# waczjoan/gaussian-mesh-splatting

Hardware: AMD Instinct MI355X
Metric: train iters/s (fwd+bwd raster) @800×800, 300k Gaussians; HBM GB/s vs roofline (higher is better)
Workload: dtype f32

## Files before the change

### gaussian-mesh-splatting_amd/csrc/binning.hip

```cpp
#include "gms_blend.h"
#include "gms_common.h"
#include "gms_forward.h"

namespace gms {

constexpr int SORT_RUN = 1024;
constexpr int SORT_RUNS_PER_TILE = 8;
constexpr int SORT_BIG_CHUNK = SORT_RUN * SORT_RUNS_PER_TILE;
constexpr int MP_CHUNK = 1024;

constexpr int NSCAN = 11;
constexpr int NCLASS = 6;
constexpr int SCAN_THREADS = 1024;

__device__ __forceinline__ void tile_terms(uint32_t c, uint32_t L, uint32_t t[NSCAN], int sort_np = 0)
{
    const uint32_t ns = max(1u, (c + L - 1) / L);
    t[0] = c; t[1] = ns; t[2] = ns > 1 ? ns : 0;
    const uint32_t r = c % L;
    t[3] = c / L;
    t[4] = r * 4 >= 3 * L ? 1u : 0u;
    t[5] = (r * 4 < 3 * L && r * 2 >= L) ? 1u : 0u;
    t[6] = (r * 2 < L && r * 4 >= L) ? 1u : 0u;
    t[7] = (r * 4 < L && r != 0) ? 1u : 0u;
// ... 177 lines not shown
    if (lane == WAVE - 1) s_wave[wave] = incl;
    __syncthreads();
    uint32_t pre = incl - sum;
    for (int w = 0; w < wave; w++) pre += s_wave[w];
#pragma unroll
    for (int k = 0; k < 16; k++)
        if (k < per && b + k < e) { s_off[b + k] = pre; pre += c[k]; }
    if (tid == BLOCK - 1) s_off[T] = pre;
    __syncthreads();
}

struct InlineScanLds {
    uint32_t chunk[NSCAN][BLOCK];
    uint32_t wave_tot[NSCAN][BLOCK / WAVE];
    uint32_t total[NSCAN];
    uint32_t wave_deep[BLOCK / WAVE];
    uint32_t deepest;
};

__device__ __forceinline__ void inline_scan_build(const uint32_t *count, int T, uint32_t L, int sort_np, InlineScanLds &S)
{
    const int tid = threadIdx.x, lane = tid & 63, wave = tid >> 6;
    const int per = (T + BLOCK - 1) / BLOCK;
    const int b = min(T, tid * per), e = min(T, b + per);
    uint32_t run[NSCAN];
    uint32_t deepest = 0;
#pragma unroll
    for (int k = 0; k < NSCAN; k++) run[k] = 0;
    for (int t = b; t < e; t++) {
        uint32_t q[NSCAN];
        tile_terms(count[t], L, q, sort_np);
        deepest = max(deepest, q[0]);
#pragma unroll
        for (int k = 0; k < NSCAN; k++) run[k] += q[k];
    }
    for (int d = 32; d >= 1; d >>= 1) deepest = max(deepest, (uint32_t)__shfl_xor((int)deepest, d));
    if (lane == 0) S.wave_deep[wave] = deepest;
    uint32_t incl[NSCAN];
#pragma unroll
    for (int k = 0; k < NSCAN; k++) {
        incl[k] = wave_incl_scan_u32(run[k], lane);
        if (lane == WAVE - 1) S.wave_tot[k][wave] = incl[k];
    }
    __syncthreads();
#pragma unroll
    for (int k = 0; k < NSCAN; k++) {
        uint32_t pre = incl[k] - run[k];
        for (int w = 0; w < wave; w++) pre += S.wave_tot[k][w];
        S.chunk[k][tid] = pre;
    }
    if (tid == 0) {
#pragma unroll
        for (int k = 0; k < NSCAN; k++) S.total[k] = S.wave_tot[k][0] + S.wave_tot[k][1] + S.wave_tot[k][2] + S.wave_tot[k][3];
        S.deepest = max(max(S.wave_deep[0], S.wave_deep[1]), max(S.wave_deep[2], S.wave_deep[3]));
    }
    __syncthreads();
}

struct InlineScanArgs {
    const uint32_t *count;
    uint32_t *offset, *unit_first, *mseg_first, *class_first, *scan_out;
    uint32_t L;
};

template <bool INLINE>
__global__ void __launch_bounds__(BLOCK) emit_instances_kernel(int P, int gx, int gy, const int *radii, GeomState geom,
                                                               const uint32_t *tile_offset, uint32_t *tile_cursor,
                                                               uint64_t *keys, uint64_t capacity, unsigned emit_blocks, FillUnitsArgs fu,
                                                               int32_t *host_slot, int32_t seq, const uint32_t *scan_out, InlineScanArgs is)
{
    constexpr int OFFW = INLINE ? INLINE_SCAN_MAX_T + 4 : 0;
    __shared__ uint32_t smem[OFFW + 3 * TT_SLOTS + BLOCK / WAVE];
    static_assert(sizeof(InlineScanLds) <= sizeof(uint32_t) * (INLINE_SCAN_MAX_T + 4 + 3 * TT_SLOTS), "spare blocks alias the emit blocks' LDS");
    uint32_t *s_off = smem, *s_wave = smem + OFFW + 3 * TT_SLOTS;
    const unsigned nspare = gridDim.x - emit_blocks;
    const bool spare = INLINE ? blockIdx.x < nspare : blockIdx.x >= emit_blocks;
    const unsigned spare_idx = INLINE ? blockIdx.x : blockIdx.x - emit_blocks;
    const unsigned emit_idx = INLINE ? blockIdx.x - nspare : blockIdx.x;
    if (spare) {
        if (INLINE) {
            InlineScanLds &S = *reinterpret_cast<InlineScanLds *>(smem);
            const int T = fu.T;
            inline_scan_build(is.count, T, is.L, fu.sort_np, S);
            const int t = (int)spare_idx * BLOCK + (int)threadIdx.x;
            if (spare_idx == 0 && threadIdx.x == 0) {
                is.scan_out[0] = S.total[0]; is.scan_out[1] = S.deepest; is.scan_out[2] = S.total[1]; is.scan_out[3] = is.L;
                if (host_slot) publish_counts(host_slot, seq, S.total[0], S.deepest, S.total[1]);
                is.offset[T] = S.total[0]; is.unit_first[T] = S.total[1]; is.mseg_first[T] = S.total[2];
#pragma unroll
                for (int k = 0; k < NCLASS + 2; k++) is.class_first[k * (T + 1) + T] = S.total[3 + k];
            }
            if (t < T) {
                const int per = (T + BLOCK - 1) / BLOCK;
                const int c0 = t / per;
                uint32_t pre[NSCAN], tot[NSCAN];
#pragma unroll
                for (int k = 0; k < NSCAN; k++) { pre[k] = S.chunk[k][c0]; tot[k] = S.total[k]; }
                for (int u = c0 * per; u < t; u++) {
                    uint32_t q[NSCAN];
                    tile_terms(is.count[u], is.L, q, fu.sort_np);
#pragma unroll
                    for (int k = 0; k < NSCAN; k++) pre[k] += q[k];
                }
                is.offset[t] = pre[0]; is.unit_first[t] = pre[1]; is.mseg_first[t] = pre[2];
#pragma unroll
                for (int k = 0; k < NCLASS + 2; k++) is.class_first[k * (T + 1) + t] = pre[3 + k];
                fill_units_tile(fu, t, is.count[t], is.L, pre, tot);
            }
            return;
        }
        if (spare_idx == 0 && threadIdx.x == 0 && host_slot) publish_counts(host_slot, seq, scan_out[0], scan_out[1], scan_out[2]);
        fill_units(fu, (int)spare_idx);
        return;
    }
    if (INLINE) { inline_offsets(is.count, fu.T, s_off, s_wave); tile_offset = s_off; }
    const int i = (int)emit_idx * BLOCK + threadIdx.x;
    const ushort4 rc = i < P ? geom.rect[i] : make_ushort4(0, 0, 0, 0);
    const uint32_t dbits = i < P ? __float_as_uint(geom.depth[i]) : 0u;
    const int minx = rc.x, miny = rc.y, maxx = rc.z, maxy = rc.w;
    const int rw = maxx - minx;
    const int area = rw * (maxy - miny);
    const uint64_t key = area > 0 ? (((uint64_t)dbits << 32) | (uint32_t)i) : 0ull;
    (void)radii; (void)gy;
    const bool small = area <= SMALL_AREA;
    const int lane = threadIdx.x & 63;
    int cx = minx, cy = miny;
    int *tt_key = reinterpret_cast<int *>(smem + OFFW);
    uint32_t *tt_cnt = smem + OFFW + TT_SLOTS, *tt_base = smem + OFFW + 2 * TT_SLOTS;
    for (int q = threadIdx.x; q < TT_SLOTS; q += BLOCK) { tt_key[q] = -1; tt_cnt[q] = 0; }
    __syncthreads();
    if (small) {
        for (int k = 0; k < area; k++) {
            const int sl = tt_insert(tt_key, cy * gx + cx);
            if (sl >= 0) atomicAdd(&tt_cnt[sl], 1u);
            if (++cx == maxx) { cx = minx; cy++; }
        }
    }
    __syncthreads();
    for (int q = threadIdx.x; q < TT_SLOTS; q += BLOCK)
        if (tt_key[q] >= 0) {
            tt_base[q] = tile_offset[tt_key[q]] + atomicAdd(&tile_cursor[tt_key[q]], tt_cnt[q]);
            tt_cnt[q] = 0;
        }
    __syncthreads();
    if (small) {
        cx = minx; cy = miny;
        for (int k = 0; k < area; k++) {
            const int t = cy * gx + cx;
            const int sl = tt_find(tt_key, t);
            const uint64_t slot = sl >= 0 ? (uint64_t)tt_base[sl] + atomicAdd(&tt_cnt[sl], 1u)
                                          : (uint64_t)tile_offset[t] + atomicAdd(&tile_cursor[t], 1u);
            if (slot < capacity) keys[slot] = key;
            if (++cx == maxx) { cx = minx; cy++; }
        }
    }
    uint64_t big = __ballot(!small);
    while (big) {
        const int src = __builtin_ctzll(big);
        big &= big - 1;
        const int bminx = __builtin_amdgcn_readlane(minx, src), bminy = __builtin_amdgcn_readlane(miny, src);
        const int brw = __builtin_amdgcn_readlane(rw, src), barea = __builtin_amdgcn_readlane(area, src);
        const uint32_t klo = (uint32_t)__builtin_amdgcn_readlane((int)(uint32_t)key, src);
        const uint32_t khi = (uint32_t)__builtin_amdgcn_readlane((int)(uint32_t)(key >> 32), src);
        const uint64_t bkey = ((uint64_t)khi << 32) | klo;
        for (int k = lane; k < barea; k += WAVE) {
            const int ty = k / brw, tx = k - ty * brw;
            const int t = (bminy + ty) * gx + bminx + tx;
            const uint64_t slot = (uint64_t)tile_offset[t] + atomicAdd(&tile_cursor[t], 1u);
            if (slot < capacity) keys[slot] = bkey;
        }
    }
}

__device__ __forceinline__ void ce(uint64_t &x, uint64_t &y)
{
    if (x > y) { uint64_t t = x; x = y; y = t; }
}


constexpr int WAVE_SPAN = 128;

template <int THREADS>
__device__ __forceinline__ void stage_sync(int span, int &prev_span)
{
    if (span > WAVE_SPAN || prev_span > WAVE_SPAN) __syncthreads();
    else wave_sync();
    prev_span = span;
}

template <int THREADS>
__device__ void lds_bitonic(uint64_t *s, int m, int k0, int j0, bool first_mirror, int tid)
{
    int prev = 1 << 30;
    for (int k = k0, lk = 31 - __builtin_clz(k0); k <= m; k <<= 1, lk++) {
        const int hk = k >> 1;
        if (k > k0 || first_mirror) {
            stage_sync<THREADS>(k, prev);
            for (int i = tid; i < (m >> 1); i += THREADS) {
                const int blk = i >> (lk - 1), off = i & (hk - 1);
                const int lo = (blk << lk) + off, hi = (blk << lk) + k - 1 - off;
                ce(s[lo], s[hi]);
            }
        }
        int j = (k > k0 || first_mirror) ? (k >> 2) : j0;
        for (int lj = j > 0 ? 31 - __builtin_clz(j) : 0; j >= 1; j >>= 1, lj--) {
            stage_sync<THREADS>(2 * j, prev);
            for (int i = tid; i < (m >> 1); i += THREADS) {
                const int lo = ((i >> lj) << (lj + 1)) + (i & (j - 1));
                ce(s[lo], s[lo + j]);
            }
        }
    }
    __syncthreads();
}


enum { SORT_SINGLE = 0, SORT_LDS, SORT_MERGEPATH, SORT_FALLBACK };

__host__ __device__ __forceinline__ int sort_passes(uint64_t n)
{
    const uint64_t runs = (n + SORT_RUN - 1) / SORT_RUN;
    int q = 0;
    while ((1ull << q) < runs) q++;
    return q;
}

__device__ __forceinline__ int sort_class(uint64_t n, int passes_launched, int &q)
{
    q = 0;
    if (n <= (uint64_t)SORT_RUN) return SORT_SINGLE;
    q = sort_passes(n);
    if (q <= passes_launched) return SORT_MERGEPATH;
    return n <= (uint64_t)SORT_BIG_CHUNK ? SORT_LDS : SORT_FALLBACK;
}

template <int CTRL>
__device__ __forceinline__ uint64_t dpp64(uint64_t v)
{
    const int lo = __builtin_amdgcn_update_dpp(0, (int)(uint32_t)v, CTRL, 0xf, 0xf, false);
    const int hi = __builtin_amdgcn_update_dpp(0, (int)(uint32_t)(v >> 32), CTRL, 0xf, 0xf, false);
    return ((uint64_t)(uint32_t)hi << 32) | (uint32_t)lo;
}
template <int ML>
__device__ __forceinline__ uint64_t lane_xor64(uint64_t v)
{
    if (ML == 1) return dpp64<0xB1>(v);
    if (ML == 2) return dpp64<0x4E>(v);
    if (ML == 3) return dpp64<0x1B>(v);
    if (ML == 4) return dpp64<0x1B>(dpp64<0x141>(v));
    if (ML == 7) return dpp64<0x141>(v);
    if (ML == 8) return dpp64<0x128>(v);
    if (ML == 15) return dpp64<0x140>(v);
    const int lo = __shfl_xor((int)(uint32_t)v, ML), hi = __shfl_xor((int)(uint32_t)(v >> 32), ML);
    return ((uint64_t)(uint32_t)hi << 32) | (uint32_t)lo;
}

template <int M>
__device__ __forceinline__ void sort_step(uint64_t (&k)[4], int t, uint64_t *lds)
{
    constexpr int MR = M & 3, ML = (M >> 2) & 63, MW = M >> 8;
    constexpr int TOP = M >= 512 ? 512 : M >= 256 ? 256 : M >= 128 ? 128 : M >= 64 ? 64 : M >= 32 ? 32 : M >= 16 ? 16 : M >= 8 ? 8 : M >= 4 ? 4 : M >= 2 ? 2 : 1;
    if (ML == 0 && MW == 0) {
        if (MR == 1) { ce(k[0], k[1]); ce(k[2], k[3]); }
        else if (MR == 2) { ce(k[0], k[2]); ce(k[1], k[3]); }
        else { ce(k[0], k[3]); ce(k[1], k[2]); }
        return;
    }
    uint64_t p[4];
    if (MW != 0) {
        __syncthreads();
#pragma unroll
        for (int r = 0; r < 4; r++) lds[4 * t + r] = k[r];
        __syncthreads();
#pragma unroll
        for (int r = 0; r < 4; r++) p[r] = lds[(4 * t + r) ^ M];
    } else {
#pragma unroll
        for (int r = 0; r < 4; r++) p[r] = lane_xor64<ML>(k[r ^ MR]);
    }
    const bool keep_min = ((4 * t) & TOP) == 0;
#pragma unroll
    for (int r = 0; r < 4; r++) {
        const bool less = p[r] < k[r];
        k[r] = (less == keep_min) ? p[r] : k[r];
    }
}
template <int J>
__device__ __forceinline__ void sort_half_cleaners(uint64_t (&k)[4], int t, uint64_t *lds)
{
    if constexpr (J >= 1) {
        sort_step<J>(k, t, lds);
        sort_half_cleaners<J / 2>(k, t, lds);
    }
}
template <int K>
__device__ __forceinline__ void sort_level(uint64_t (&k)[4], int t, uint64_t *lds)
{
    sort_step<K - 1>(k, t, lds);
    sort_half_cleaners<K / 4>(k, t, lds);
}

__global__ void __launch_bounds__(256) tile_presort_reg_kernel(const uint32_t *tile_offset, const uint32_t *run_total, const uint2 *run_tab,
                                                           uint32_t max_runs, uint64_t *keys, uint64_t *tmp, uint64_t capacity,
                                                           int passes_launched, uint32_t *zero_count, int T)
{
    __shared__ uint64_t s[SORT_RUN];
    const int tid = threadIdx.x;
    if (zero_count)
        for (int q = (int)blockIdx.x * 256 + tid; q < T; q += (int)gridDim.x * 256) zero_count[q] = 0u;
    if (blockIdx.x >= run_total[0] || blockIdx.x >= max_runs) return;
    const uint2 tr = run_tab[blockIdx.x];
    const uint64_t beg = tile_offset[tr.x], end64 = tile_offset[tr.x + 1];
    if (end64 > capacity) return;
    const long n = (long)(end64 - beg);
    int q;
    const int cls = sort_class((uint64_t)n, passes_launched, q);
    if (cls == SORT_FALLBACK) return;
    uint64_t *dst_base = (cls == SORT_MERGEPATH && (q & 1)) ? tmp : keys;
    const long c0 = (long)tr.y * SORT_RUN;
    const int cn = (int)min((long)SORT_RUN, n - c0);
    const uint64_t *g = keys + beg + c0;
    uint64_t *d = dst_base + beg + c0;
    if (cn <= 1) { if (cn == 1 && tid == 0) d[0] = g[0]; return; }
    int m = 2;
    while (m < cn) m <<= 1;
    uint64_t k[4];
#pragma unroll
    for (int r = 0; r < 4; r++) k[r] = 4 * tid + r < cn ? g[4 * tid + r] : ~0ull;
    sort_level<2>(k, tid, s);
    sort_level<4>(k, tid, s);
    if (m >= 8) sort_level<8>(k, tid, s);
    if (m >= 16) sort_level<16>(k, tid, s);
    if (m >= 32) sort_level<32>(k, tid, s);
    if (m >= 64) sort_level<64>(k, tid, s);
    if (m >= 128) sort_level<128>(k, tid, s);
    if (m >= 256) sort_level<256>(k, tid, s);
    if (m >= 512) sort_level<512>(k, tid, s);
    if (m >= 1024) sort_level<1024>(k, tid, s);
#pragma unroll
    for (int r = 0; r < 4; r++)
        if (4 * tid + r < cn) d[4 * tid + r] = k[r];
}

template <typename PA, typename PB>
__device__ __forceinline__ int co_rank(int o, PA A, int la, PB B, int lb)
{
    int lo = max(0, o - lb), hi = min(o, la);
    while (lo < hi) {
        const int mid = (lo + hi) >> 1;
        if (A[mid] < B[o - mid - 1]) lo = mid + 1;
        else hi = mid;
    }
    return lo;
}

__device__ __forceinline__ int co_rank_wave(int o, const uint64_t *A, int la, const uint64_t *B, int lb)
{
    const int lane = threadIdx.x & 63;
    int lo = max(0, o - lb), hi = min(o, la);
    while (lo < hi) {
        const int step = (hi - lo + 63) / 64;
        const int mid = lo + lane * step;
        const bool need_more = mid < hi && A[mid] < B[o - mid - 1];
        const int cnt = __builtin_popcountll(__ballot(need_more));
        const int nlo = cnt > 0 ? lo + (cnt - 1) * step + 1 : lo;
        const int nhi = (cnt < 64 && lo + cnt * step < hi) ? lo + cnt * step : hi;
        lo = nlo; hi = nhi;
    }
    return lo;
}

__global__ void __launch_bounds__(256) tile_mergepath_kernel(const uint32_t *tile_offset, const uint32_t *deep_first, const uint2 *deep_tab,
                                                             uint32_t max_deep, uint64_t *keys, uint64_t *tmp, uint64_t capacity,
                                                             int passes_launched, int pass)
{
    __shared__ uint64_t s[MP_CHUNK];
    __shared__ int s_rank[2];
    const int tid = threadIdx.x;
    if (blockIdx.x >= deep_first[0] || blockIdx.x >= max_deep) return;
    const uint2 tc = deep_tab[blockIdx.x];
    const uint64_t beg = tile_offset[tc.x], end64 = tile_offset[tc.x + 1];
    if (end64 > capacity) return;
    const long n = (long)(end64 - beg);
    int q;
    if (sort_class((uint64_t)n, passes_launched, q) != SORT_MERGEPATH || pass >= q) return;
    const bool src_is_tmp = ((q - pass) & 1) != 0;
    const uint64_t *src = (src_is_tmp ? tmp : keys) + beg;
    uint64_t *dst = (src_is_tmp ? keys : tmp) + beg;
    const long w = (long)SORT_RUN << pass;
    const long j0 = (long)tc.y * MP_CHUNK;
    const long base = (j0 / (2 * w)) * (2 * w);
    const long a1 = min(n, base + w), b1 = min(n, base + 2 * w);
    const int la = (int)(a1 - base), lb = (int)(b1 - a1);
    const uint64_t *A = src + base, *B = src + a1;
    const int o0 = (int)(j0 - base), o1 = (int)min((long)(o0 + MP_CHUNK), (long)(la + lb));
    if (tid < 64) { const int r = co_rank_wave(o0, A, la, B, lb); if (tid == 0) s_rank[0] = r; }
    else if (tid < 128) { const int r = co_rank_wave(o1, A, la, B, lb); if (tid == 64) s_rank[1] = r; }
    __syncthreads();
    const int ra0 = s_rank[0], ra1 = s_rank[1];
    const int rb0 = o0 - ra0, rb1 = o1 - ra1;
    const int na = ra1 - ra0, nb = rb1 - rb0;
    for (int i = tid; i < na; i += 256) s[i] = A[ra0 + i];
    for (int i = tid; i < nb; i += 256) s[na + i] = B[rb0 + i];
    __syncthreads();
    const int cnt = o1 - o0;
    const int lo = tid * 4;
    if (lo < cnt) {
        const uint64_t *LA = s, *LB = s + na;
        int ia = co_rank(lo, LA, na, LB, nb), ib = lo - ia;
        uint64_t out[4];
        const int m = min(4, cnt - lo);
        for (int k = 0; k < m; k++) {
            const bool takeA = ib >= nb || (ia < na && LA[ia] < LB[ib]);
            out[k] = takeA ? LA[ia++] : LB[ib++];
        }
        for (int k = 0; k < m; k++) dst[base + o0 + lo + k] = out[k];
    }
}

__global__ void __launch_bounds__(1024) tile_merge_kernel(const uint32_t *tile_offset, const uint32_t *multi_total, const uint32_t *multi_tab,
                                                          uint32_t max_multi, uint64_t *keys, uint64_t capacity, int passes_launched)
{
    constexpr int THREADS = 1024, CHUNK = SORT_BIG_CHUNK;
    __shared__ uint64_t s[CHUNK];
    const int tid = threadIdx.x;
    if (blockIdx.x >= multi_total[0] || blockIdx.x >= max_multi) return;
    const uint32_t tile = multi_tab[blockIdx.x];
    const uint64_t beg = tile_offset[tile], end64 = tile_offset[tile + 1];
    if (end64 > capacity) return;
    const long n = (long)(end64 - beg);
    int q;
    const int cls = sort_class((uint64_t)n, passes_launched, q);
    if (cls == SORT_SINGLE || cls == SORT_MERGEPATH) return;
    uint64_t *g = keys + beg;
    long np2 = 2;
    while (np2 < n) np2 <<= 1;
    const uint64_t INF = ~0ull;

    if (cls == SORT_LDS) {
        const int m = (int)np2;
        for (int i = tid; i < m; i += THREADS) s[i] = i < n ? g[i] : INF;
        __syncthreads();
        const int K = m / THREADS;
        for (int w = SORT_RUN; w < m; w <<= 1) {
            const int o = tid * K;
            const int base = (o / (2 * w)) * (2 * w);
            const uint64_t *LA = s + base, *LB = s + base + w;
            const int lo = o - base;
            int ia = co_rank(lo, LA, w, LB, w), ib = lo - ia;
            uint64_t out[8];
#pragma unroll
            for (int k = 0; k < 8; k++) {
                if (k < K) {
                    const bool takeA = ib >= w || (ia < w && LA[ia] < LB[ib]);
                    out[k] = takeA ? LA[ia++] : LB[ib++];
                }
            }
            __syncthreads();
#pragma unroll
            for (int k = 0; k < 8; k++)
                if (k < K) s[o + k] = out[k];
            __syncthreads();
        }
        for (int i = tid; i < n; i += THREADS) g[i] = s[i];
        return;
    }
    for (long c = 0; c < n; c += CHUNK) {
        for (int i = tid; i < CHUNK; i += THREADS) s[i] = (c + i) < n ? g[c + i] : INF;
        lds_bitonic<THREADS>(s, CHUNK, 2, 0, true, tid);
        for (int i = tid; i < CHUNK; i += THREADS)
            if (c + i < n) g[c + i] = s[i];
        __syncthreads();
    }
    for (long k = 2L * CHUNK; k <= np2; k <<= 1) {
        const long hk = k >> 1;
        for (long i = tid; i < (np2 >> 1); i += THREADS) {
            long blk = i / hk, off = i - blk * hk;
            long lo = blk * k + off, hi = blk * k + k - 1 - off;
            if (hi < n) { uint64_t x = g[lo], y = g[hi]; if (x > y) { g[lo] = y; g[hi] = x; } }
        }
        __syncthreads();
        for (long j = k >> 2; j >= CHUNK; j >>= 1) {
            for (long i = tid; i < (np2 >> 1); i += THREADS) {
                long lo = 2 * j * (i / j) + (i % j), hi = lo + j;
                if (hi < n) { uint64_t x = g[lo], y = g[hi]; if (x > y) { g[lo] = y; g[hi] = x; } }
            }
            __syncthreads();
        }
        for (long c = 0; c < n; c += CHUNK) {
            for (int i = tid; i < CHUNK; i += THREADS) s[i] = (c + i) < n ? g[c + i] : INF;
            lds_bitonic<THREADS>(s, CHUNK, CHUNK, CHUNK >> 1, false, tid);
            for (int i = tid; i < CHUNK; i += THREADS)
                if (c + i < n) g[c + i] = s[i];
            __syncthreads();
        }
    }
}

int merge_path_passes(uint32_t deepest, uint32_t headroom)
{
    return deepest > (uint32_t)SORT_BIG_CHUNK ? sort_passes((uint64_t)deepest + headroom) : 0;
}

bool inline_scan_fits(int T, int P) { return T <= INLINE_SCAN_MAX_T && (P + BLOCK - 1) / BLOCK <= 1536; }

int32_t launch_tile_scan(const BinningFrame &f, bool debug, hipStream_t stream)
{
    const ImageState &img = f.img;
    GMS_LAUNCH(GMS_K_TILE_SCAN, stream, tile_scan_kernel<<<1, SCAN_THREADS, 0, stream>>>(img.tile_count, img.tile_offset, img.tile_cursor,
                                                                                   img.unit_first, img.mseg_first, img.class_first, f.T, f.frame_L,
                                                                                   f.pub_slot, f.seq, f.scan_np, img.scan_out));
    GMS_KERNEL_CHECK(debug, stream, "tile_scan");
    return GMS_OK;
}

int32_t launch_emit_sort(const BinningFrame &f, const BinningState &bin, uint64_t capacity, uint32_t max_units, bool inl, int fill_np, int sort_np,
                         bool *presort_enqueued, bool debug, hipStream_t stream)
{
    const ImageState &img = f.img;
    const int T = f.T;
    const uint32_t max_deep = (uint32_t)BinningState::n_deep((size_t)capacity, (size_t)T);
    const uint32_t max_multi = (uint32_t)BinningState::n_multi((size_t)capacity);
    FillUnitsArgs fu;
    fu.class_first = img.class_first; fu.offset = img.tile_offset; fu.mseg_first = img.mseg_first;
    fu.unit_tile = bin.unit_tile; fu.deep_tab = bin.deep_tab; fu.multi_tab = bin.multi_tab;
    fu.max_multi = max_multi; fu.T = T; fu.sort_np = fill_np; fu.scan_out = img.scan_out; fu.max_units = max_units;
    fu.max_deep = max_deep;
    const unsigned pblocks = (unsigned)((f.P + BLOCK - 1) / BLOCK), fblocks = (unsigned)((T + BLOCK - 1) / BLOCK);
    InlineScanArgs isa{img.tile_count, img.tile_offset, img.unit_first, img.mseg_first, img.class_first, img.scan_out, f.frame_L};
    *presort_enqueued = false;
    if (inl)
        GMS_LAUNCH(GMS_K_EMIT, stream, emit_instances_kernel<true><<<pblocks + fblocks, BLOCK, 0, stream>>>(f.P, f.gx, f.gy, f.radii, f.geom, img.tile_offset,
                                                                                                             img.tile_cursor, bin.keys, capacity, pblocks, fu,
                                                                                                             f.pub_slot, f.seq, img.scan_out, isa));
    else
        GMS_LAUNCH(GMS_K_EMIT, stream, emit_instances_kernel<false><<<pblocks + fblocks, BLOCK, 0, stream>>>(f.P, f.gx, f.gy, f.radii, f.geom, img.tile_offset,
                                                                                                              img.tile_cursor, bin.keys, capacity, pblocks, fu,
                                                                                                              nullptr, f.seq, img.scan_out, isa));
    GMS_KERNEL_CHECK(debug, stream, "emit_instances");
    uint64_t *sort_tmp = reinterpret_cast<uint64_t *>(bin.seg_state);
    const uint32_t *run_total = img.class_first + NCLASS * ((size_t)T + 1) + T;
    const uint32_t *multi_total = img.class_first + (NCLASS + 1) * ((size_t)T + 1) + T;
    GMS_LAUNCH(GMS_K_TILE_SORT, stream, tile_presort_reg_kernel<<<max_deep, 256, 0, stream>>>(img.tile_offset, run_total, bin.deep_tab, max_deep, bin.keys,
                                                                                             sort_tmp, capacity, sort_np, inl ? img.tile_count : nullptr, T));
    *presort_enqueued = true;
    for (int pass = 0; pass < sort_np; pass++)
        GMS_LAUNCH(GMS_K_TILE_SORT, stream, tile_mergepath_kernel<<<max_deep, 256, 0, stream>>>(img.tile_offset, run_total, bin.deep_tab, max_deep, bin.keys,
                                                                                               sort_tmp, capacity, sort_np, pass));
    GMS_LAUNCH(GMS_K_TILE_SORT, stream, tile_merge_kernel<<<max_multi, 1024, 0, stream>>>(img.tile_offset, multi_total, bin.multi_tab, max_multi, bin.keys,
                                                                                         capacity, sort_np));
    GMS_KERNEL_CHECK(debug, stream, "tile_sort");
    return GMS_OK;
}

}
```

### gaussian-mesh-splatting_amd/csrc/gms_forward.h

```cpp
#pragma once
#include "gms_common.h"

namespace gms {

constexpr int SMALL_AREA = 64;

struct PreArgs {
    int P, D, M, W, H, gx, gy;
    const float *means3D, *shs, *shs_rest, *colors, *opac, *scales, *rots, *cov3Dp, *view, *proj, *campos;
    float mod, tanx, tany;
    int aa;
    int *radii;
    uint8_t *visible;
    GeomState geom;
    uint32_t *tile_count;
    uint32_t *zero_cursor;
    uint32_t *zero_cmax;
    int T;
    GmsMeshArgs mesh;
    float *k0_xyz, *k0_scale, *k0_rot, *k0_opac;
};

int32_t launch_preprocess_forward(const PreArgs &a, const GmsPointsArgs *points, bool fused_mesh, bool fast_layout, bool debug, hipStream_t stream);

struct BinningFrame {
    int P, gx, gy, T;
    const int *radii;
    GeomState geom;
    ImageState img;
    uint32_t frame_L;
    int32_t *pub_slot;
    int32_t seq;
    int scan_np;
};

int32_t launch_tile_scan(const BinningFrame &f, bool debug, hipStream_t stream);
int32_t launch_emit_sort(const BinningFrame &f, const BinningState &bin, uint64_t capacity, uint32_t max_units, bool inline_scan, int fill_np,
                         int sort_np, bool *presort_enqueued, bool debug, hipStream_t stream);
int merge_path_passes(uint32_t deepest, uint32_t headroom);
bool inline_scan_fits(int T, int P);

}
```

### gaussian-mesh-splatting_amd/csrc/raster_forward.hip

```cpp
#include <stdarg.h>
#include <stdio.h>

#include <stdlib.h>
#include <mutex>

#include "gms_blend.h"
#include "gms_mesh.h"
#include "gms_points.h"
#include <atomic>
#include <vector>
#include <chrono>

#include "gms_common.h"
#include "gms_project.h"
#include "gms_forward.h"

namespace gms {

static thread_local char g_err[512] = "";
void set_error(const char *fmt, ...)
{
    va_list ap;
    va_start(ap, fmt);
    vsnprintf(g_err, sizeof(g_err), fmt, ap);
// ... 27 lines not shown
    int32_t *slots = nullptr;
    int32_t seq_counter = 0;
    uint32_t defer_counter = 0;
    std::vector<Counters> counters;
    std::vector<FrameState> frames;
    uint32_t last_deepest = 0;
    int64_t last_launched_units = 0;
    int32_t last_used_micro = 0;
};
static thread_local ThreadState t_state;

constexpr int DEFER_SLOTS = 16, SLOT_WORDS = 16;
static int32_t *pinned_slot(int index = 0)
{
    int32_t *&slot = t_state.slots;
    if (!slot) {
        if (hipHostMalloc((void **)&slot, 64 * (1 + DEFER_SLOTS), hipHostMallocPortable | hipHostMallocMapped) != hipSuccess) slot = nullptr;
        else { for (int k = 0; k < SLOT_WORDS * (1 + DEFER_SLOTS); k++) slot[k] = 0; }
    }
    return slot ? slot + SLOT_WORDS * index : nullptr;
}

static std::atomic<int64_t> g_wait_ns{0}, g_wait_calls{0};

static int32_t wait_for_count(int32_t *slot, int32_t seq, hipStream_t stream, int64_t *N)
{
    const auto t0 = std::chrono::steady_clock::now();
    struct Tally {
        std::chrono::steady_clock::time_point t0;
        ~Tally() { g_wait_ns += std::chrono::duration_cast<std::chrono::nanoseconds>(std::chrono::steady_clock::now() - t0).count(); g_wait_calls++; }
    } tally{t0};
    const unsigned long long *hs = reinterpret_cast<const unsigned long long *>(slot);
    const unsigned long long tag = (unsigned long long)(uint32_t)seq;
    auto ready = [&]() {
        return (__atomic_load_n(&hs[0], __ATOMIC_ACQUIRE) >> 32) == tag && (__atomic_load_n(&hs[1], __ATOMIC_ACQUIRE) >> 32) == tag &&
               (__atomic_load_n(&hs[2], __ATOMIC_ACQUIRE) >> 32) == tag;
    };
    for (uint32_t spins = 0;; spins++) {
        if (ready()) break;
        __builtin_ia32_pause();
        if ((spins & 0xffffu) == 0xffffu &&
            std::chrono::duration<double>(std::chrono::steady_clock::now() - t0).count() > 10.0) {
            GMS_HIP_CHECK(hipStreamSynchronize(stream));
            if (!ready()) {
                set_error("tile_scan did not publish the instance count");
                return GMS_ERR_HIP;
            }
            break;
        }
    }
    *N = (int64_t)(uint32_t)(__atomic_load_n(&hs[0], __ATOMIC_RELAXED) & 0xffffffffull);
    return GMS_OK;
}
static uint32_t unit_count(const int32_t *slot)
{
    return (uint32_t)(__atomic_load_n(reinterpret_cast<const unsigned long long *>(slot) + 2, __ATOMIC_RELAXED) & 0xffffffffull);
}
static uint32_t deepest_tile(const int32_t *slot)
{
    return (uint32_t)(__atomic_load_n(reinterpret_cast<const unsigned long long *>(slot) + 1, __ATOMIC_RELAXED) & 0xffffffffull);
}

int micro_setting()
{
    static int m = -2;
    if (m == -2) { const char *e = getenv("GMS_MICRO"); m = e ? (atoi(e) != 0 ? 1 : 0) : (GMS_MICRO_DEFAULT ? -1 : 0); }
    return m;
}
bool micro_mode() { return micro_setting() != 0; }
bool use_micro(uint64_t capacity, int T) { const int m = micro_setting(); return m == 1 || (m < 0 && capacity <= 512ull * (uint64_t)T); }

uint32_t seg_len_forced()
{
    static int64_t L = -1;
    if (L < 0) {
        uint32_t v = 0;
        if (const char *e = getenv("GMS_SEG_LEN")) { v = (uint32_t)atoi(e); if (v < 64) v = 64; v = (v + 63u) / 64u * 64u; }
        if (micro_mode()) { if (v == 0) v = SEG_LEN_MICRO; if (v > 256u) v = 256u; }
        L = v;
    }
    return (uint32_t)L;
}
uint32_t seg_len_min() { const uint32_t f = seg_len_forced(); return f ? f : SEG_LEN_SHALLOW; }
static uint32_t seg_len_for_frame(uint64_t capacity_hint, int T)
{
    const uint32_t f = seg_len_forced();
    if (f == 0 || getenv("GMS_SEG_LEN") || micro_setting() == 1) return f;
    return capacity_hint > (uint64_t)SEG_VERY_DEEP_PER_TILE * (uint64_t)T ? SEG_LEN_VERY_DEEP : f;
}

uint32_t unit_run()
{
    static uint32_t R = 0;
    if (R == 0) {
        uint32_t v = 4;
        if (const char *e = getenv("GMS_UNIT_RUN")) v = (uint32_t)atoi(e);
        R = 1;
        while (R * 2 <= v && R < 64) R *= 2;
    }
    return R;
}

static bool inline_scan_setting()
{
    static const bool on = [] { const char *e = getenv("GMS_INLINE_SCAN"); return e ? atoi(e) != 0 : true; }();
    return on;
}

}

using namespace gms;

extern "C" int32_t gms_abi_version(void) { return GMS_ABI_VERSION; }
extern "C" const char *gms_last_error(void) { return gms::g_err; }
extern "C" size_t gms_geom_bytes(int32_t P) { return GeomState::bytes((size_t)(P > 0 ? P : 1)); }
extern "C" size_t gms_image_bytes(int32_t w, int32_t h) { return ImageState::bytes((size_t)w, (size_t)h); }
extern "C" size_t gms_image_n_contrib_offset(int32_t w, int32_t h)
{
    char *const base = reinterpret_cast<char *>(uintptr_t(1) << 20);
    ImageState s = ImageState::carve(base, (size_t)w, (size_t)h);
    return (size_t)(reinterpret_cast<char *>(s.n_contrib) - base);
}
extern "C" size_t gms_image_counts_offset(int32_t w, int32_t h)
{
    char *const base = reinterpret_cast<char *>(uintptr_t(1) << 20);
    ImageState s = ImageState::carve(base, (size_t)w, (size_t)h);
    return (size_t)(reinterpret_cast<char *>(s.scan_out) - base);
}
static FrameState *frame_state(const FrameKey &key)
{
    std::vector<FrameState> &frames = t_state.frames;
    for (auto &f : frames) if (f.key == key) return &f;
    if (frames.size() >= 64) frames.erase(frames.begin());
    frames.push_back({key, 0u, 0u});
    return &frames.back();
}
static uint32_t decayed_units(uint32_t hint, uint32_t units) { return max(units, (uint32_t)(0.97 * hint)); }

struct HintMail { FrameKey key; uint32_t deepest, units; };
static std::mutex g_mail_mu;
static std::vector<HintMail> g_mail;
static void post_mail(const FrameKey &key, uint32_t deepest, uint32_t units)
{
    std::lock_guard<std::mutex> lk(g_mail_mu);
    for (auto &m : g_mail)
        if (m.key == key) { m.deepest = deepest; m.units = units; return; }
    if (g_mail.size() >= 64) g_mail.erase(g_mail.begin());
    g_mail.push_back({key, deepest, units});
}
static void take_mail(FrameState *fs)
{
    std::lock_guard<std::mutex> lk(g_mail_mu);
    for (size_t k = 0; k < g_mail.size(); k++)
        if (g_mail[k].key == fs->key) {
            fs->deepest_seen = g_mail[k].deepest;
            fs->units_hint = decayed_units(fs->units_hint, g_mail[k].units);
            g_mail.erase(g_mail.begin() + (long)k);
            return;
        }
}

static int32_t take_counts(int32_t *slot, int32_t seq, hipStream_t stream, FrameState *fs, int64_t *N, uint32_t *units)
{
    const int32_t rc = wait_for_count(slot, seq, stream, N);
    if (rc != GMS_OK) return rc;
    fs->deepest_seen = t_state.last_deepest = deepest_tile(slot);
    *units = unit_count(slot);
    fs->units_hint = decayed_units(fs->units_hint, *units);
    return GMS_OK;
}

extern "C" int64_t gms_last_launched_units(void) { return t_state.last_launched_units; }
extern "C" int32_t gms_last_used_micro(void) { return t_state.last_used_micro; }
extern "C" size_t gms_binning_bytes(int64_t n, int32_t w, int32_t h)
{
    const size_t T = (size_t)((w + TILE - 1) / TILE) * (size_t)((h + TILE - 1) / TILE);
    return BinningState::bytes((size_t)(n > 0 ? n : 0), T, seg_len_min(), micro_mode());
}

static bool aligned16(const void *p) { return (((uintptr_t)p) & 15u) == 0; }
static bool sh_fast_layout(const GmsRasterForwardArgs *A)
{
    return A->shs && A->M == 16 && aligned16(A->shs) && aligned16(A->shs_rest) &&
           (A->mesh || A->points || A->cov3D_precomp || aligned16(A->rotations));
}

static int32_t validate_forward(const GmsRasterForwardArgs *A)
{
    if (!A || A->P < 0 || A->width <= 0 || A->height <= 0 || !A->out_color || !A->out_invdepth || !A->background) {
        set_error("gms_rasterize_forward: invalid sizes or null output/background pointer");
        return GMS_ERR_INVALID_ARGUMENT;
    }
    const GmsMeshArgs *mesh = A->mesh;
    const GmsPointsArgs *points = A->points;
    if (mesh && points) { set_error("gms_rasterize_forward: set at most one of mesh / points"); return GMS_ERR_INVALID_ARGUMENT; }
    if (A->P == 0) return GMS_OK;
    const bool fused = mesh || points;
    if (fused) {
        const int32_t rc = mesh ? check_mesh_args(mesh, false) : check_points_args(points);
        if (rc != GMS_OK) return rc;
        if (mesh) {
            const int outs = (A->mesh_out_xyz != nullptr) + (A->mesh_out_scaling_act != nullptr) + (A->mesh_out_rotation_unit != nullptr) +
                             (A->mesh_out_opacity_act != nullptr);
            if (outs != 0 && (outs != 4 || !aligned16(A->mesh_out_rotation_unit))) {
                set_error("gms_rasterize_forward: mesh_out_* must be all NULL (forward-only frame) or all set (rotation_unit 16-byte aligned)");
                return GMS_ERR_INVALID_ARGUMENT;
            }
        }
        const bool complete = mesh ? mesh->P == (int64_t)A->P && mesh->vertices && mesh->faces && mesh->_alpha && mesh->_scale && mesh->_opacity &&
                                         (mesh->splats_per_face > 0 || mesh->splat_face)
                                   : points->P == (int64_t)A->P && points->_opacity;
        if (!complete || !A->shs || !A->shs_rest || A->M != 16 || A->D < 0 || A->D > 3 || A->colors_precomp || A->cov3D_precomp ||
            !aligned16(A->shs) || !aligned16(A->shs_rest)) {
            set_error("gms_rasterize_forward: the fused %s input needs a complete %s (P equal, _opacity set), split degree-3 SH "
                      "storage (shs + shs_rest, M = 16, active degree 0 .. 3, 16-byte aligned) and no precomputed colours / covariances",
                      mesh ? "mesh" : "points", mesh ? "GmsMeshArgs" : "GmsPointsArgs");
            return GMS_ERR_INVALID_ARGUMENT;
        }
    } else {
        if ((A->shs == nullptr) == (A->colors_precomp == nullptr)) { set_error("provide exactly one of shs / colors_precomp"); return GMS_ERR_INVALID_ARGUMENT; }
        const bool sr = A->scales && A->rotations;
        if (sr == (A->cov3D_precomp != nullptr) || (!sr && (A->scales || A->rotations))) {
            set_error("provide exactly one of (scales, rotations) / cov3D_precomp");
            return GMS_ERR_INVALID_ARGUMENT;
        }
    }
    if ((!fused && (!A->means3D || !A->opacities)) || !A->viewmatrix || !A->projmatrix || !A->campos || !A->radii || !A->geom_alloc ||
        !A->binning_alloc || !A->image_alloc) {
        set_error("gms_rasterize_forward: null input pointer or callback");
        return GMS_ERR_INVALID_ARGUMENT;
    }
    if (!fused && A->shs && (A->D < 0 || A->D > 3 || (A->D + 1) * (A->D + 1) > A->M)) {
        set_error("SH degree %d needs %d coefficients but M = %d (degrees 0..3 supported)", A->D, (A->D + 1) * (A->D + 1), A->M);
        return GMS_ERR_INVALID_ARGUMENT;
    }
    if (A->shs_rest && !sh_fast_layout(A)) { set_error("split SH storage (shs_rest) needs M == 16 and 16-byte aligned pointers"); return GMS_ERR_INVALID_ARGUMENT; }
    if (A->no_host_wait && A->binning_capacity_hint <= 0) { set_error("no_host_wait needs a binning capacity hint (render the shape once without it first)"); return GMS_ERR_INVALID_ARGUMENT; }
    return GMS_OK;
}

static int32_t claim_tile_counters(int device, hipStream_t stream, int T, Counters **out)
{
    std::vector<Counters> &counters = t_state.counters;
    Counters *ctr = nullptr;
    for (auto &c : counters) if (c.device == device && c.stream == stream) ctr = &c;
    if (!ctr) { counters.push_back({device, stream, nullptr, 0, true}); ctr = &counters.back(); }
    if (ctr->cap < (size_t)T) {
        if (ctr->buf) (void)hipFree(ctr->buf);
        ctr->buf = nullptr; ctr->cap = 0;
        GMS_HIP_CHECK(hipMalloc((void **)&ctr->buf, (size_t)T * 4));
        ctr->cap = (size_t)T; ctr->dirty = true;
    }
    if (ctr->dirty) GMS_HIP_CHECK(hipMemsetAsync(ctr->buf, 0, ctr->cap * 4, stream));
    ctr->dirty = true;
    *out = ctr;
    return GMS_OK;
}

static PreArgs pre_args(const GmsRasterForwardArgs *A, const GeomState &geom, const ImageState &img, int gx, int gy, bool inline_scan)
{
    PreArgs pa{};
    pa.P = A->P; pa.D = A->D; pa.M = A->M; pa.W = A->width; pa.H = A->height; pa.gx = gx; pa.gy = gy;
    pa.shs = A->shs; pa.shs_rest = A->shs_rest; pa.colors = A->colors_precomp; pa.view = A->viewmatrix;
    pa.proj = A->projmatrix; pa.campos = A->campos; pa.mod = A->scale_modifier; pa.tanx = A->tan_fovx;
    pa.tany = A->tan_fovy; pa.aa = A->antialiasing; pa.radii = A->radii; pa.visible = A->visible; pa.geom = geom; pa.tile_count = img.tile_count;
    if (!A->mesh && !A->points) {
        pa.means3D = A->means3D; pa.opac = A->opacities; pa.scales = A->scales; pa.rots = A->rotations; pa.cov3Dp = A->cov3D_precomp;
    }
    if (A->mesh) {
        pa.mesh = *A->mesh;
        pa.k0_xyz = A->mesh_out_xyz; pa.k0_scale = A->mesh_out_scaling_act; pa.k0_rot = A->mesh_out_rotation_unit; pa.k0_opac = A->mesh_out_opacity_act;
    }
    pa.zero_cursor = inline_scan ? img.tile_cursor : nullptr; pa.T = gx * gy;
    pa.zero_cmax = micro_mode() ? img.tile_cmax : nullptr;
    return pa;
}

struct ForwardTail {
    BinningFrame f;
    int W, H;
    BlendFwdOut bo;
    uint32_t L;
    bool inline_scan, debug;
    const FrameState *fs;
    Counters *ctr;
    hipStream_t stream;
    bool scanned = false;
    bool scratch_short = false;

    int32_t run(void *bin_mem, uint64_t capacity, bool exact_fit, uint32_t *launched_units)
    {
        const int T = f.T;
        BinningState bin = BinningState::carve(bin_mem, (size_t)capacity, (size_t)T, L);
        const uint32_t mu = (uint32_t)BinningState::n_units((size_t)capacity, (size_t)T, L);
        uint32_t mu_launch = mu;
        if (!exact_fit && fs->units_hint > 0) mu_launch = min(mu, fs->units_hint + fs->units_hint / 4u + 64u);
        *launched_units = blend_grid_units(mu_launch);
        const bool inl = inline_scan && !scanned;
        scanned = true;
        const int fill_np = scratch_short ? 0 : f.scan_np;
        if ((uint64_t)BinningState::n_slots((size_t)capacity, L) * 7u * TILE_PIX * 4u < capacity * 8u) scratch_short = true;
        const int sort_np = scratch_short ? 0 : f.scan_np;
        bool presort_enqueued = false;
        const int32_t rc = launch_emit_sort(f, bin, capacity, mu, inl, fill_np, sort_np, &presort_enqueued, debug, stream);
        if (inl && presort_enqueued) ctr->dirty = false;
        if (rc != GMS_OK) return rc;
        const BlendGrid g = make_blend_grid(W, H, f.img, bin, capacity, L);
        bool used_micro = false;
        const int32_t brc = launch_compositing_forward(g, bo, f.frame_L, mu_launch, debug, stream, &used_micro);
        t_state.last_used_micro = used_micro ? 1 : 0;
        return brc;
    }
};

static void *alloc_binning(const GmsRasterForwardArgs *A, uint64_t capacity, int T, uint32_t L)
{
    void *mem = A->binning_alloc(A->binning_ctx, BinningState::bytes((size_t)capacity, (size_t)T, L, micro_mode()));
    if (!mem) set_error("binning allocation callback returned NULL");
    return mem;
}

extern "C" int64_t gms_rasterize_forward(const GmsRasterForwardArgs *A, void *stream_)
{
    gms::TraceRange trace_range("gms_rasterize_forward");
    hipStream_t stream = (hipStream_t)stream_;
    g_err[0] = 0;
    if (const int32_t rc = validate_forward(A)) return rc;
    const int P = A->P, W = A->width, H = A->height;
    const int gx = (W + TILE - 1) / TILE, gy = (H + TILE - 1) / TILE, T = gx * gy;
    const size_t HW = (size_t)W * H;
    const bool debug = A->debug != 0;
    if (P == 0) {
        fill_background_kernel<<<(unsigned)((HW + 255) / 256), 256, 0, stream>>>(W, H, A->background, A->out_color, A->out_invdepth);
        GMS_KERNEL_CHECK(A->debug, stream, "fill_background");
        return 0;
    }

    void *geom_mem = A->geom_alloc(A->geom_ctx, GeomState::bytes((size_t)P));
    void *img_mem = A->image_alloc(A->image_ctx, ImageState::bytes((size_t)W, (size_t)H));
    if (!geom_mem || !img_mem) { set_error("scratch allocation callback returned NULL"); return GMS_ERR_ALLOC; }
    GeomState geom = GeomState::carve(geom_mem, (size_t)P);
    ImageState img = ImageState::carve(img_mem, (size_t)W, (size_t)H);
    int device = 0;
    GMS_HIP_CHECK(hipGetDevice(&device));
    ThreadState &ts = t_state;
    Counters *ctr = nullptr;
    if (const int32_t rc = claim_tile_counters(device, stream, T, &ctr)) return rc;
    img.tile_count = ctr->buf;
    FrameState *fs = frame_state({device, stream, W, H, P});
    take_mail(fs);

    const uint64_t hint = A->binning_capacity_hint > 0 ? (uint64_t)A->binning_capacity_hint : 0;
    const uint32_t frame_L = seg_len_for_frame(hint, T);
    const bool inline_scan = inline_scan_setting() && hint > 0 && frame_L != 0 && inline_scan_fits(T, P);
    const PreArgs pa = pre_args(A, geom, img, gx, gy, inline_scan);
    if (const int32_t rc = launch_preprocess_forward(pa, A->points, A->mesh != nullptr, sh_fast_layout(A), debug, stream)) return rc;
    const uint32_t L = seg_len_min();
    const bool defer = A->count_ticket_out != nullptr && hint > 0 && !A->no_host_wait;
    const int slot_index = defer ? 1 + (int)(ts.defer_counter++ % (uint32_t)DEFER_SLOTS) : 0;
    int32_t *slot = pinned_slot(slot_index);
    if (!slot) { set_error("hipHostMalloc for the read-back slot failed"); return GMS_ERR_HIP; }
    const int32_t seq = (ts.seq_counter = ts.seq_counter == 0x7fffffff ? 1 : ts.seq_counter + 1);
    const BinningFrame bf{P, gx, gy, T, A->radii, geom, img, frame_L, A->no_host_wait ? nullptr : slot, seq,
                          merge_path_passes(fs->deepest_seen, fs->deepest_seen / 4)};
    if (!inline_scan) {
        if (const int32_t rc = launch_tile_scan(bf, debug, stream)) return rc;
        ctr->dirty = false;
    }
    const BlendFwdOut bo{geom.rec, A->background, img.final_T, img.n_contrib, A->out_color, A->out_invdepth};
    ForwardTail tail{bf, W, H, bo, L, inline_scan, debug, fs, ctr, stream};
    uint32_t launched_units = 0;
    if (A->no_host_wait || defer) {
        void *bin_mem = alloc_binning(A, hint, T, L);
        if (!bin_mem) return GMS_ERR_ALLOC;
        if (const int32_t rc = tail.run(bin_mem, hint, false, &launched_units)) return rc;
        ts.last_launched_units = (int64_t)launched_units;
        if (defer) {
            A->count_ticket_out[0] = (int64_t)(uintptr_t)slot;
            A->count_ticket_out[1] = (int64_t)seq;
        }
        if (A->num_units_out) *A->num_units_out = 0;
        return (int64_t)hint;
    }
    int64_t N;
    uint32_t units_seen = 0;
    if (hint > 0) {
        void *bin_mem = alloc_binning(A, hint, T, L);
        if (!bin_mem) return GMS_ERR_ALLOC;
        if (const int32_t rc = tail.run(bin_mem, hint, false, &launched_units)) return rc;
        ts.last_launched_units = (int64_t)launched_units;
        if (const int32_t rc = take_counts(slot, seq, stream, fs, &N, &units_seen)) return rc;
        if ((uint64_t)N <= hint && units_seen > launched_units) {
            GMS_HIP_CHECK(hipMemsetAsync(img.tile_cursor, 0, (size_t)T * 4, stream));
            if (const int32_t rc = tail.run(bin_mem, hint, true, &launched_units)) return rc;
        }
        if ((uint64_t)N > hint) {
            bin_mem = alloc_binning(A, (uint64_t)N, T, L);
            if (!bin_mem) return GMS_ERR_ALLOC;
            GMS_HIP_CHECK(hipMemsetAsync(img.tile_cursor, 0, (size_t)T * 4, stream));
            if (const int32_t rc = tail.run(bin_mem, (uint64_t)N, true, &launched_units)) return rc;
        }
    } else {
        if (const int32_t rc = take_counts(slot, seq, stream, fs, &N, &units_seen)) return rc;
        const uint64_t cap = (uint64_t)(N > 0 ? N : 1);
        void *bin_mem = alloc_binning(A, cap, T, L);
        if (!bin_mem) return GMS_ERR_ALLOC;
        if (const int32_t rc = tail.run(bin_mem, cap, true, &launched_units)) return rc;
    }
    if (A->num_units_out) *A->num_units_out = (int64_t)units_seen;
    return N;
}

extern "C" int64_t gms_rasterize_forward_counts(const int64_t *ticket, int32_t width, int32_t height, int32_t P, int64_t *num_units_out,
                                                int64_t *deepest_tile_out, void *stream_)
{
    gms::TraceRange trace_range("gms_rasterize_forward_counts");
    hipStream_t stream = (hipStream_t)stream_;
    set_error("%s", "");
    if (!ticket || ticket[0] == 0 || ticket[1] <= 0 || ticket[1] > 0x7fffffffll) {
        set_error("gms_rasterize_forward_counts: not a ticket of a deferred forward");
        return GMS_ERR_INVALID_ARGUMENT;
    }
    int32_t *slot = reinterpret_cast<int32_t *>((uintptr_t)ticket[0]);
    const int32_t seq = (int32_t)ticket[1];
    const unsigned long long tag0 = __atomic_load_n(reinterpret_cast<const unsigned long long *>(slot), __ATOMIC_ACQUIRE) >> 32;
    if (tag0 != 0ull && (int32_t)(uint32_t)tag0 - seq > 0) {
        set_error("gms_rasterize_forward_counts: ticket expired (more than %d deferred forwards outstanding on the forward's host thread)", DEFER_SLOTS);
        return GMS_ERR_INVALID_ARGUMENT;
    }
    int64_t N = 0;
    const int32_t rc = wait_for_count(slot, seq, stream, &N);
    if (rc != GMS_OK) return rc;
    const uint32_t units = unit_count(slot), deepest = deepest_tile(slot);
    int device = 0;
    GMS_HIP_CHECK(hipGetDevice(&device));
    post_mail({device, stream, width, height, P}, deepest, units);
    t_state.last_deepest = deepest;
    if (num_units_out) *num_units_out = (int64_t)units;
    if (deepest_tile_out) *deepest_tile_out = (int64_t)deepest;
    return N;
}

extern "C" int64_t gms_last_deepest_tile(void) { return (int64_t)t_state.last_deepest; }

extern "C" void gms_wait_stats(double *total_ms, int64_t *calls, int32_t reset)
{
    if (total_ms) *total_ms = (double)g_wait_ns.load() * 1e-6;
    if (calls) *calls = g_wait_calls.load();
    if (reset) { g_wait_ns = 0; g_wait_calls = 0; }
}

extern "C" int32_t gms_mark_visible(int32_t P, const float *means3D, const float *viewmatrix, const float *projmatrix,
                                    uint8_t *present, void *stream_)
{
    (void)projmatrix;
    hipStream_t stream = (hipStream_t)stream_;
    g_err[0] = 0;
    if (P < 0 || (P > 0 && (!means3D || !viewmatrix || !present))) {
        set_error("gms_mark_visible: invalid argument");
        return GMS_ERR_INVALID_ARGUMENT;
    }
    if (P == 0) return GMS_OK;
    mark_visible_kernel<<<(unsigned)((P + 255) / 256), 256, 0, stream>>>(P, means3D, viewmatrix, present);
    GMS_KERNEL_CHECK(0, stream, "mark_visible");
    return GMS_OK;
}
```

Baseline: 3034.

## Merge LDS-class tile runs by rank across blocks with persistent work-list kernel

For tiles whose keys fit in LDS, the presort now writes its sorted 1024-key runs to scratch. A new merge path then places each key directly by binary-searching its rank in the other runs, so each run of a tile can be handled by its own work item rather than one block doing repeated merge-path passes per tile. The merge kernel becomes a persistent grid of at most 256 blocks that builds a shared work list of (tile, run) items and loops over it. This raises parallelism for deep tiles, at the cost of an extra scratch round trip, reloading every run of the tile into LDS for each run item, and a launch capped at 256 blocks.

```diff
diff --git a/gaussian-mesh-splatting_amd/csrc/binning.hip b/gaussian-mesh-splatting_amd/csrc/binning.hip
--- a/gaussian-mesh-splatting_amd/csrc/binning.hip
+++ b/gaussian-mesh-splatting_amd/csrc/binning.hip
@@ -503,7 +503,7 @@
 
 __global__ void __launch_bounds__(256) tile_presort_reg_kernel(const uint32_t *tile_offset, const uint32_t *run_total, const uint2 *run_tab,
                                                            uint32_t max_runs, uint64_t *keys, uint64_t *tmp, uint64_t capacity,
-                                                           int passes_launched, uint32_t *zero_count, int T)
+                                                           int passes_launched, bool by_rank, uint32_t *zero_count, int T)
 {
     __shared__ uint64_t s[SORT_RUN];
     const int tid = threadIdx.x;
@@ -517,7 +517,7 @@
     int q;
     const int cls = sort_class((uint64_t)n, passes_launched, q);
     if (cls == SORT_FALLBACK) return;
-    uint64_t *dst_base = (cls == SORT_MERGEPATH && (q & 1)) ? tmp : keys;
+    uint64_t *dst_base = ((cls == SORT_MERGEPATH && (q & 1)) || (cls == SORT_LDS && by_rank)) ? tmp : keys;
     const long c0 = (long)tr.y * SORT_RUN;
     const int cn = (int)min((long)SORT_RUN, n - c0);
     const uint64_t *g = keys + beg + c0;
@@ -619,26 +619,66 @@
     }
 }
 
-__global__ void __launch_bounds__(1024) tile_merge_kernel(const uint32_t *tile_offset, const uint32_t *multi_total, const uint32_t *multi_tab,
-                                                          uint32_t max_multi, uint64_t *keys, uint64_t capacity, int passes_launched)
+template <int R>
+__device__ __forceinline__ int rank_in_other_runs(const uint64_t *s, int run, uint64_t key)
+{
+    const uint64_t *a[R - 1];
+    int p[R - 1];
+#pragma unroll
+    for (int o = 0; o < R - 1; o++) { a[o] = s + (o < run ? o : o + 1) * SORT_RUN; p[o] = 0; }
+#pragma unroll
+    for (int step = SORT_RUN / 2; step >= 1; step >>= 1) {
+#pragma unroll
+        for (int o = 0; o < R - 1; o++) p[o] += a[o][p[o] + step - 1] < key ? step : 0;
+    }
+    int below = 0;
+#pragma unroll
+    for (int o = 0; o < R - 1; o++) below += p[o] + (a[o][p[o]] < key ? 1 : 0);
+    return below;
+}
+
+__device__ __forceinline__ bool merge_item_has_work(const uint32_t *tile_offset, uint32_t tile, int run, uint64_t capacity, int passes_launched,
+                                                    bool by_rank)
+{
+    const uint64_t beg = tile_offset[tile], end64 = tile_offset[tile + 1];
+    if (end64 > capacity) return false;
+    int q;
+    const int cls = sort_class(end64 - beg, passes_launched, q);
+    if (cls == SORT_LDS && by_rank) return (uint64_t)run * SORT_RUN < end64 - beg;
+    return (cls == SORT_LDS || cls == SORT_FALLBACK) && run == 0;
+}
+
+__device__ __forceinline__ void merge_run_by_rank(uint64_t *s, const uint64_t *src, uint64_t *g, int n, int run)
+{
+    const int tid = threadIdx.x;
+    const int R = (n + SORT_RUN - 1) / SORT_RUN;
+    for (int i = tid; i < R * SORT_RUN; i += 1024) s[i] = i < n ? src[i] : ~0ull;
+    __syncthreads();
+    const int own = run * SORT_RUN + tid;
+    if (own >= n) return;
+    const uint64_t key = s[own];
+    int below = 0;
+    switch (R) {
+    case 2: below = rank_in_other_runs<2>(s, run, key); break;
+    case 3: below = rank_in_other_runs<3>(s, run, key); break;
+    case 4: below = rank_in_other_runs<4>(s, run, key); break;
+    case 5: below = rank_in_other_runs<5>(s, run, key); break;
+    case 6: below = rank_in_other_runs<6>(s, run, key); break;
+    case 7: below = rank_in_other_runs<7>(s, run, key); break;
+    default: below = rank_in_other_runs<8>(s, run, key); break;
+    }
+    g[tid + below] = key;
+}
+
+__device__ __forceinline__ void merge_tile_one_block(uint64_t *s, uint64_t *g, long n, bool runs_in_lds)
 {
     constexpr int THREADS = 1024, CHUNK = SORT_BIG_CHUNK;
-    __shared__ uint64_t s[CHUNK];
     const int tid = threadIdx.x;
-    if (blockIdx.x >= multi_total[0] || blockIdx.x >= max_multi) return;
-    const uint32_t tile = multi_tab[blockIdx.x];
-    const uint64_t beg = tile_offset[tile], end64 = tile_offset[tile + 1];
-    if (end64 > capacity) return;
-    const long n = (long)(end64 - beg);
-    int q;
-    const int cls = sort_class((uint64_t)n, passes_launched, q);
-    if (cls == SORT_SINGLE || cls == SORT_MERGEPATH) return;
-    uint64_t *g = keys + beg;
+    const uint64_t INF = ~0ull;
     long np2 = 2;
     while (np2 < n) np2 <<= 1;
-    const uint64_t INF = ~0ull;
-
-    if (cls == SORT_LDS) {
+
+    if (runs_in_lds) {
         const int m = (int)np2;
         for (int i = tid; i < m; i += THREADS) s[i] = i < n ? g[i] : INF;
         __syncthreads();
@@ -698,6 +738,46 @@
     }
 }
 
+__device__ __forceinline__ void merge_tile_run(uint64_t *s, const uint32_t *tile_offset, uint32_t tile, int run, uint64_t *keys,
+                                               const uint64_t *tmp, int passes_launched, bool by_rank)
+{
+    const uint64_t beg = tile_offset[tile];
+    const long n = (long)(tile_offset[tile + 1] - beg);
+    int q;
+    const int cls = sort_class((uint64_t)n, passes_launched, q);
+    if (cls == SORT_LDS && by_rank) merge_run_by_rank(s, tmp + beg, keys + beg, (int)n, run);
+    else merge_tile_one_block(s, keys + beg, n, cls == SORT_LDS);
+}
+
+constexpr int MERGE_BLOCKS = 256;
+
+__global__ void __launch_bounds__(1024) tile_merge_kernel(const uint32_t *tile_offset, const uint32_t *multi_total, const uint32_t *multi_tab,
+                                                          uint32_t max_multi, uint64_t *keys, const uint64_t *tmp, uint64_t capacity,
+                                                          int passes_launched, bool by_rank)
+{
+    constexpr int THREADS = 1024;
+    __shared__ uint64_t s[SORT_BIG_CHUNK];
+    __shared__ uint32_t s_work[THREADS], s_nwork;
+    const uint32_t entries = min(multi_total[0], max_multi), items = entries * SORT_RUNS_PER_TILE;
+    for (uint32_t first = blockIdx.x; first < items; first += THREADS * gridDim.x) {
+        if (threadIdx.x == 0) s_nwork = 0;
+        __syncthreads();
+        const uint32_t item = first + threadIdx.x * gridDim.x;
+        if (item < items) {
+            const uint32_t tile = multi_tab[item % entries], run = item / entries;
+            if (merge_item_has_work(tile_offset, tile, (int)run, capacity, passes_launched, by_rank))
+                s_work[atomicAdd(&s_nwork, 1u)] = tile * SORT_RUNS_PER_TILE + run;
+        }
+        __syncthreads();
+        const uint32_t nwork = s_nwork;
+        for (uint32_t w = 0; w < nwork; w++) {
+            const uint32_t work = (uint32_t)__builtin_amdgcn_readfirstlane((int)s_work[w]);
+            merge_tile_run(s, tile_offset, work / SORT_RUNS_PER_TILE, (int)(work % SORT_RUNS_PER_TILE), keys, tmp, passes_launched, by_rank);
+            __syncthreads();
+        }
+    }
+}
+
 int merge_path_passes(uint32_t deepest, uint32_t headroom)
 {
     return deepest > (uint32_t)SORT_BIG_CHUNK ? sort_passes((uint64_t)deepest + headroom) : 0;
@@ -716,7 +796,7 @@
 }
 
 int32_t launch_emit_sort(const BinningFrame &f, const BinningState &bin, uint64_t capacity, uint32_t max_units, bool inl, int fill_np, int sort_np,
-                         bool *presort_enqueued, bool debug, hipStream_t stream)
+                         bool scratch_fits, bool *presort_enqueued, bool debug, hipStream_t stream)
 {
     const ImageState &img = f.img;
     const int T = f.T;
@@ -743,13 +823,15 @@
     const uint32_t *run_total = img.class_first + NCLASS * ((size_t)T + 1) + T;
     const uint32_t *multi_total = img.class_first + (NCLASS + 1) * ((size_t)T + 1) + T;
     GMS_LAUNCH(GMS_K_TILE_SORT, stream, tile_presort_reg_kernel<<<max_deep, 256, 0, stream>>>(img.tile_offset, run_total, bin.deep_tab, max_deep, bin.keys,
-                                                                                             sort_tmp, capacity, sort_np, inl ? img.tile_count : nullptr, T));
+                                                                                             sort_tmp, capacity, sort_np, scratch_fits,
+                                                                                             inl ? img.tile_count : nullptr, T));
     *presort_enqueued = true;
     for (int pass = 0; pass < sort_np; pass++)
         GMS_LAUNCH(GMS_K_TILE_SORT, stream, tile_mergepath_kernel<<<max_deep, 256, 0, stream>>>(img.tile_offset, run_total, bin.deep_tab, max_deep, bin.keys,
                                                                                                sort_tmp, capacity, sort_np, pass));
-    GMS_LAUNCH(GMS_K_TILE_SORT, stream, tile_merge_kernel<<<max_multi, 1024, 0, stream>>>(img.tile_offset, multi_total, bin.multi_tab, max_multi, bin.keys,
-                                                                                         capacity, sort_np));
+    const uint32_t merge_blocks = min(max_multi * (uint32_t)SORT_RUNS_PER_TILE, (uint32_t)MERGE_BLOCKS);
+    GMS_LAUNCH(GMS_K_TILE_SORT, stream, tile_merge_kernel<<<merge_blocks, 1024, 0, stream>>>(img.tile_offset, multi_total, bin.multi_tab, max_multi,
+                                                                                            bin.keys, sort_tmp, capacity, sort_np, scratch_fits));
     GMS_KERNEL_CHECK(debug, stream, "tile_sort");
     return GMS_OK;
 }
diff --git a/gaussian-mesh-splatting_amd/csrc/gms_forward.h b/gaussian-mesh-splatting_amd/csrc/gms_forward.h
--- a/gaussian-mesh-splatting_amd/csrc/gms_forward.h
+++ b/gaussian-mesh-splatting_amd/csrc/gms_forward.h
@@ -36,7 +36,7 @@
 
 int32_t launch_tile_scan(const BinningFrame &f, bool debug, hipStream_t stream);
 int32_t launch_emit_sort(const BinningFrame &f, const BinningState &bin, uint64_t capacity, uint32_t max_units, bool inline_scan, int fill_np,
-                         int sort_np, bool *presort_enqueued, bool debug, hipStream_t stream);
+                         int sort_np, bool scratch_fits, bool *presort_enqueued, bool debug, hipStream_t stream);
 int merge_path_passes(uint32_t deepest, uint32_t headroom);
 bool inline_scan_fits(int T, int P);
 
diff --git a/gaussian-mesh-splatting_amd/csrc/raster_forward.hip b/gaussian-mesh-splatting_amd/csrc/raster_forward.hip
--- a/gaussian-mesh-splatting_amd/csrc/raster_forward.hip
+++ b/gaussian-mesh-splatting_amd/csrc/raster_forward.hip
@@ -353,7 +353,7 @@
         if ((uint64_t)BinningState::n_slots((size_t)capacity, L) * 7u * TILE_PIX * 4u < capacity * 8u) scratch_short = true;
         const int sort_np = scratch_short ? 0 : f.scan_np;
         bool presort_enqueued = false;
-        const int32_t rc = launch_emit_sort(f, bin, capacity, mu, inl, fill_np, sort_np, &presort_enqueued, debug, stream);
+        const int32_t rc = launch_emit_sort(f, bin, capacity, mu, inl, fill_np, sort_np, !scratch_short, &presort_enqueued, debug, stream);
         if (inl && presort_enqueued) ctr->dirty = false;
         if (rc != GMS_OK) return rc;
         const BlendGrid g = make_blend_grid(W, H, f.img, bin, capacity, L);
```

Result: faster. 3090, median of 6 (+1.8%).
